# JustKshitijD/genomicsbench_palisade

Hardware: AMD Instinct MI355X
Metric: GCUPS (phmm) + Mreads/s (fmi) on 'large' set at 1/2/4/8 MI355X (higher is better)
Workload: dtype f32+f64 (phmm), int64 (fmi), int32/f64 (chain), int32 (bsw); 1 GPU; phmm large: 64 batches, 755118 testcases, 47.634 G cells per step (whole job); all 755118 testcases; 36.0% of rank 0's testcases on the f64 fallback; parallelism=shard1 (strong scaling, no data-path collective)

## Files before the change

### genomicsbench_palisade_amd/csrc/phmm.hip

```cpp
#include <hip/hip_runtime.h>

#include <algorithm>
#include <cmath>
#include <cstdint>
#include <cstdlib>
#include <chrono>
#include <cstring>
#include <functional>
#include <future>
#include <limits>
#include <mutex>
#include <string>
#include <unordered_map>
#include <thread>
#include <type_traits>
#include <vector>

#include "../../include/gb_phmm.h"
#include "gb_common.h"
#include "gb_common_wave.h"

namespace {

constexpr int kWave = 64;
constexpr int kLdsHaplen = 9400;
constexpr int kMaxHaplen = 65535;
constexpr int kBndPad = 72;
constexpr int kRecPad = 16;
constexpr int kQualTab = 128;
constexpr int kStackRows = 2048;
constexpr int kPlanBuckets = 128;
constexpr int kPlanCount = 8, kPlanCursor = kPlanCount + kPlanBuckets, kPlanTotal = kPlanCursor + kPlanBuckets;
constexpr int kCountWords = kPlanTotal + 8;
constexpr int kPredSampled = kPlanTotal + 1, kPredSamplePred = kPlanTotal + 2, kPredPredicted = kPlanTotal + 3;
constexpr int kPredConfirmed = kPlanTotal + 4, kPredRedone = kPlanTotal + 5, kRedoUnits = kPlanTotal + 6;
constexpr int kRedoNext = kPlanTotal + 7;
static_assert(kRedoNext < kCountWords, "counter words");
constexpr int kMaxF64Parts = 8;
constexpr int kM2M = ((127 * 128) >> 1) + 128;

constexpr int kMaxQual = 254;
constexpr double kJacTol = 8.0;
constexpr double kJacStep = 0.0001;
#define GB_JAC_INV_STEP (1.0 / kJacStep)
constexpr int kJacSize = (int)(kJacTol / kJacStep) + 1;

template <typename T>
struct HostTables {
  T ph2pr[kQualTab];
  T one_minus[kQualTab];
  T div3[kQualTab];
  T m2m[kM2M];
  T init_const;
  T log10_init;
};

template <typename T>
static int fast_round(T d) {
  return (d > (T)0.0) ? (int)(d + (T)0.5) : (int)(d - (T)0.5);
}

template <typename T>
static T log10sum(const std::vector<T> &jac, T small, T big) {
  if (small > big) std::swap(small, big);
  T diff = big - small;
  if (diff >= (T)kJacTol) return big;
  int ind = fast_round<T>((T)(diff * (T)GB_JAC_INV_STEP));
  return big + jac[ind];
}

template <typename T>
static void build_tables(HostTables<T> &t) {
  std::vector<T> jac(kJacSize);
  for (int k = 0; k < kJacSize; k++) jac[k] = (T)(log10(1.0 + pow(10.0, -((double)k) * kJacStep)));
  const double inv_ln10 = 1.0 / log(10);
  std::vector<T> m2m_full(((kMaxQual + 1) * (kMaxQual + 2)) >> 1);
  for (int i = 0, off = 0; i <= kMaxQual; off += ++i)
    for (int j = 0; j <= i; j++) {
      double s = log10sum<T>(jac, (T)(-0.1 * i), (T)(-0.1 * j));
      double l = log1p(-std::min(1.0, pow(10, s))) * inv_ln10;
      m2m_full[off + j] = (T)(pow(10, l));
    }
  for (int k = 0; k < kM2M; k++) t.m2m[k] = m2m_full[k];
  for (int x = 0; x < kQualTab; x++) {
    if constexpr (sizeof(T) == 4)
      t.ph2pr[x] = powf(10.f, -((float)x) / 10.f);
    else
      t.ph2pr[x] = pow(10.0, -((double)x) / 10.0);
    t.one_minus[x] = (T)1.0 - t.ph2pr[x];
    t.div3[x] = t.ph2pr[x] / (T)3.0;
  }
  if constexpr (sizeof(T) == 4) {
    t.init_const = ldexpf(1.f, 120);
    t.log10_init = log10f(t.init_const);
  } else {
    t.init_const = ldexp(1.0, 1020);
    t.log10_init = log10(t.init_const);
  }
}

static uint8_t base_code(char ch) {
  switch ((uint8_t)ch) {
    case 'A': return 0;
    case 'C': return 1;
    case 'T': return 2;
    case 'G': return 3;
    case 'N': return 4;
    default: return 0;
  }
}
static uint8_t read_match_mask(uint8_t rc) { return rc == 4 ? 0x1F : (uint8_t)((1u << rc) | 0x10); }

constexpr double kExitGrowthMax = 2.0;
constexpr uint8_t kMayExit = 0x80;
static double exit_growth(const HostTables<float> &t, const uint8_t *rec, int R) {
  const double inf = std::numeric_limits<double>::infinity();
  double G = 1.0;
  for (int k = 0; k + 1 < R; k++) {
    const int qd = rec[3 * R + k] & 127, qc = rec[4 * R + k] & 127;
    const int ni = rec[2 * R + k + 1] & 127, nd = rec[3 * R + k + 1] & 127, nc = rec[4 * R + k + 1] & 127;
    const int mn = std::min(ni, nd), mx = std::max(ni, nd);
    const double nMM = t.m2m[((mx * (mx + 1)) >> 1) + mn], nMX = t.ph2pr[ni];
    const double nGAPM = t.one_minus[nc], nXX = t.ph2pr[nc];
    const double pYY = t.ph2pr[qc], leak = (double)t.ph2pr[qd] * nGAPM;
    if (leak > 0 && pYY >= 1.0) return inf;
    const double gM = nMM + nMX + (leak > 0 ? leak / (1.0 - pYY) : 0.0), gX = nGAPM + nXX;
    const double g = std::max(gM, gX);
    if (g > 1.0) G *= g;
    if (G > 1e30) return inf;
  }
  return G;
}

constexpr double kCertMax = 2.0;
constexpr uint8_t kMayPredict = 0x80;
struct CertTab {
  double q[kQualTab];
  double p[kQualTab];
  double c[kQualTab];
  double m[kM2M];
};
static void build_cert_tab(const HostTables<float> &tf, const HostTables<double> &td, CertTab &T) {
  auto ratio = [](float f, double d) {
    return d > 0 ? std::max(1.0, (double)f / d) : (f > 0 ? std::numeric_limits<double>::infinity() : 1.0);
  };
  for (int x = 0; x < kQualTab; x++) {
    T.q[x] = std::max(ratio(tf.one_minus[x], td.one_minus[x]), ratio(tf.div3[x], td.div3[x]));
    T.p[x] = ratio(tf.ph2pr[x], td.ph2pr[x]);
    T.c[x] = std::max(T.p[x], ratio(tf.one_minus[x], td.one_minus[x]));
  }
  for (int k = 0; k < kM2M; k++) T.m[k] = ratio(tf.m2m[k], td.m2m[k]);
}
static double cert_log_rho(const CertTab &T, const uint8_t *q, const uint8_t *qi, const uint8_t *qd,
                           const uint8_t *qc, int R) {
  double rho = 1.0;
  for (int r = 0; r < R; r++) {
    const int a = q[r] & 127, i = qi[r] & 127, d = qd[r] & 127, c = qc[r] & 127;
    if (i <= 3 || d <= 3 || a == 0 || c == 0) return std::numeric_limits<double>::infinity();
    const int mn = std::min(i, d), mx = std::max(i, d), m = ((mx * (mx + 1)) >> 1) + mn;
    rho = std::max(rho, std::max(std::max(T.q[a], T.p[i]), std::max(std::max(T.p[d], T.c[c]), T.m[m])));
  }
  return std::log(rho);
}
__host__ __device__ inline double cert_K(double log_rho, int R, int C) {
  const double steps = (double)R + (double)C, D = 4.0 * steps + (double)C + 4.0;
  return exp((2.0 * steps + 2.0) * log_rho + D * 5.9604644e-8);
}

struct __attribute__((aligned(16))) TcDesc {
  uint32_t read_off;
  uint32_t hap_off;
  uint32_t dims;
  uint32_t out_idx;
};

template <typename T>
struct DevTab {
  const T *ph2pr, *one_minus, *div3, *m2m;
  T init_const;
};

template <typename T>
struct __attribute__((aligned(2 * sizeof(T)))) Brec {
  T z, w;
};

template <int (*F)(int, int)>
__device__ __forceinline__ float dpp(float v, float keep) {
  return __builtin_bit_cast(float, F(__builtin_bit_cast(int, v), __builtin_bit_cast(int, keep)));
}
template <int (*F)(int, int)>
__device__ __forceinline__ double dpp(double v, double keep) {
  long long vb = __builtin_bit_cast(long long, v), kb = __builtin_bit_cast(long long, keep);
  int lo = F((int)(vb & 0xffffffffll), (int)(kb & 0xffffffffll));
  int hi = F((int)(vb >> 32), (int)(kb >> 32));
  return __builtin_bit_cast(double, ((long long)hi << 32) | (unsigned int)lo);
}
template <int (*F)(int, int)>
__device__ __forceinline__ uint32_t dpp(uint32_t v, uint32_t keep) {
  return (uint32_t)F((int)v, (int)keep);
}

__device__ __forceinline__ float select_dist(uint32_t rmask, uint32_t h, float dmatch, float dmis) {
  uint32_t m = (uint32_t)__builtin_amdgcn_sbfe((int)rmask, h, 1);
  uint32_t r = (m & __builtin_bit_cast(uint32_t, dmatch)) | (~m & __builtin_bit_cast(uint32_t, dmis));
  return __builtin_bit_cast(float, r);
}
__device__ __forceinline__ double select_dist(uint32_t rmask, uint32_t h, double dmatch, double dmis) {
  uint32_t m;
  asm("v_bfe_i32 %0, %1, %2, 1" : "=v"(m) : "v"(rmask), "v"(h));
  const uint64_t a = __builtin_bit_cast(uint64_t, dmatch), b = __builtin_bit_cast(uint64_t, dmis);
  const uint32_t lo = (m & (uint32_t)a) | (~m & (uint32_t)b);
  const uint32_t hi = (m & (uint32_t)(a >> 32)) | (~m & (uint32_t)(b >> 32));
  return __builtin_bit_cast(double, ((uint64_t)hi << 32) | lo);
}

template <int O>
__device__ __forceinline__ float swz_xor(float v) {
  return __builtin_bit_cast(float, __builtin_amdgcn_ds_swizzle(__builtin_bit_cast(int, v), (O << 10) | 0x1F));
}
template <int O>
__device__ __forceinline__ double swz_xor(double v) {
  const long long b = __builtin_bit_cast(long long, v);
  const int lo = __builtin_amdgcn_ds_swizzle((int)(b & 0xffffffffll), (O << 10) | 0x1F);
  const int hi = __builtin_amdgcn_ds_swizzle((int)(b >> 32), (O << 10) | 0x1F);
  return __builtin_bit_cast(double, ((long long)hi << 32) | (unsigned int)lo);
}
template <typename T>
__device__ __forceinline__ T wave_sum_xor(T acc) {
  acc += __shfl_xor(acc, 32);
  acc += swz_xor<16>(acc);
  acc += swz_xor<8>(acc);
  acc += swz_xor<4>(acc);
  acc += swz_xor<2>(acc);
  acc += swz_xor<1>(acc);
  return acc;
}

__device__ __forceinline__ int fresh(int v) {
  asm volatile("" : "+v"(v));
  return v;
}

__device__ __forceinline__ uint32_t load_code(const uint8_t *p) {
  uint32_t h = *p;
  asm volatile("" : "+v"(h));
  return h;
}

template <typename T>
struct RowParams {
  T pMY, pYY, dmatch, dmis;
  T nMM, nGAPM, nGAPMx, nMX, nXX;
  uint32_t rmask;
};

template <typename T>
struct LaneState {
  T Mp, Yp, zo, wo, zd;
};

template <typename T, bool kSum, bool kWrite>
__device__ __forceinline__ void phmm_step(const Brec<T> &rec, uint32_t h, LaneState<T> &st,
// ... 609 lines not shown
      phmm_step2<T, kSum, W>(c1, h1, hb, A, B, PA, PB, sMa, sXa, sMb, sXb, wr + 1, last_lane);
      phmm_step2<T, kSum, W>(c2, h2, hb, A, B, PA, PB, sMa, sXa, sMb, sXb, wr + 2, last_lane);
      phmm_step2<T, kSum, W>(c3, h3, hb, A, B, PA, PB, sMa, sXa, sMb, sXb, wr + 3, last_lane);
    }
    for (; t < end; t++) single(t, wr_tag);
  };
  if constexpr (kWrite) {
    const int a = min(steps, kNoWrite2);
    run(0, a, std::false_type{});
    run(a, steps, std::true_type{});
  } else {
    run(0, steps, std::false_type{});
  }
}

template <typename T>
__device__ __forceinline__ void phmm_stack2(const Stack &S, const uint32_t *__restrict__ stk_tc,
                                            const TcDesc *__restrict__ descs, const uint8_t *__restrict__ pool,
                                            const DevTab<T> &tab, T *__restrict__ raw_out, uint8_t *smem_raw) {
  const int lane = threadIdx.x;
  const int C = (int)S.C;
  Brec<T> *bnd = reinterpret_cast<Brec<T> *>(smem_raw) + kRecPad;
  uint8_t *hcol = smem_raw + sizeof(Brec<T>) * (size_t)(C + kBndPad2 + kRecPad) + kCodePad2;
  const int na = (int)S.count;
  TcDesc d = {0, 0, 0, 0};
  if (lane < na) d = descs[stk_tc[S.first + lane]];
  const int rows = lane < na ? (int)(d.dims & 0xffff) + 2 : 0;
  const int incl = gb::scan_add(rows);
  const int T_rows = __builtin_amdgcn_readlane(incl, 63);
  const int e_start = incl - rows, e_R = rows - 2;
  const T init_Y = tab.init_const / (T)C;
  const uint8_t *hcode = pool + S.hap_off;
  for (int c = lane; c < C + kBndPad2; c += kWave) {
    Brec<T> b;
    b.z = (T)0;
    b.w = (T)0;
    bnd[c] = b;
  }
  for (int c = lane - kCodePad2; c < C + kBndPad2; c += kWave)
    hcol[c] = (c >= 1 && c <= C) ? hcode[c - 1] : (c == 0 ? 5 : (c < 0 ? 6 : 0));
  __syncthreads();

  const int nstripes = (T_rows + kRows2 - 1) / kRows2;
  for (int s = 0; s < nstripes; s++) {
    const int g0 = s * kRows2 + 2 * lane, g1 = g0 + 1;
    int lo = 0, hi = na - 1;
    while (__builtin_amdgcn_ballot_w64(lo < hi)) {
      const int mid = (lo + hi + 1) >> 1;
      const int sm = __shfl(e_start, mid);
      if (lo < hi) {
        if (sm <= g0) lo = mid; else hi = mid - 1;
      }
    }
    const int nxt = __shfl(e_start, min(lo + 1, kWave - 1));
    const int lob = (lo + 1 < na && nxt <= g1) ? lo + 1 : lo;
    const int sa = __shfl(e_start, lo), Ra = __shfl(e_R, lo);
    const uint32_t rda = (uint32_t)__shfl((int)d.read_off, lo), oa = (uint32_t)__shfl((int)d.out_idx, lo);
    const int sb = __shfl(e_start, lob), Rb = __shfl(e_R, lob);
    const uint32_t rdb = (uint32_t)__shfl((int)d.read_off, lob), ob = (uint32_t)__shfl((int)d.out_idx, lob);
    const int ra = g0 - sa, rb = g1 - sb;
    const bool deadA = g0 >= T_rows, deadB = g1 >= T_rows;
    RowParams<T> PA, PB;
    LaneState<T> A, B;
    const T z_top = lane == 0 ? bnd[0].z : (T)0;
    setup_row<T>(2 * lane, deadA, ra, Ra, pool + rda, tab, init_Y, z_top, PA, A);
    setup_row<T>(2 * lane + 1, deadB, rb, Rb, pool + rdb, tab, init_Y, (T)0, PB, B);
    const uint64_t pa = __builtin_amdgcn_ballot_w64(!deadA && ra == Ra + 1);
    const uint64_t pb = __builtin_amdgcn_ballot_w64(!deadB && rb == Rb + 1);
    const bool more = s < nstripes - 1;
    const int steps = more ? C + kRows2 - 1 : C + (T_rows - s * kRows2) - 1;
    T *outA = raw_out + oa, *outB = raw_out + ob;
    if (pa | pb) {
      if (more)
        phmm_stripe2<T, true, true>(steps, A, B, PA, PB, bnd, hcol, C, lane, pa, pb, outA, outB);
      else
        phmm_stripe2<T, true, false>(steps, A, B, PA, PB, bnd, hcol, C, lane, pa, pb, outA, outB);
    } else {
      phmm_stripe2<T, false, true>(steps, A, B, PA, PB, bnd, hcol, C, lane, 0, 0, outA, outB);
    }
    __syncthreads();
  }
}

template <int W>
__global__ __launch_bounds__(64) __attribute__((amdgpu_waves_per_eu(W ? W : 1, 8))) void phmm_forward2(
                                                     const Stack *__restrict__ stacks,
                                                     const uint32_t *__restrict__ stk_tc,
                                                     const TcDesc *__restrict__ descs,
                                                     const uint8_t *__restrict__ pool, DevTab<float> tab,
                                                     float *__restrict__ raw_out) {
  extern __shared__ __attribute__((aligned(16))) uint8_t smem_raw[];
  phmm_stack2<float>(stacks[blockIdx.x], stk_tc, descs, pool, tab, raw_out, smem_raw);
}

template <typename T, bool kF64Pass, bool kLong = false, bool kExit = false, bool kRedo = false>
__global__ __launch_bounds__(64) __attribute__((amdgpu_waves_per_eu(kLong ? 1 : (sizeof(T) == 4 ? 8 : 4), 8))) void phmm_forward(
    const Stack *__restrict__ stacks, int nstacks,
                                                    const uint32_t *__restrict__ stk_tc,
                                                    const TcDesc *__restrict__ descs,
                                                    const uint8_t *__restrict__ pool, DevTab<T> tab,
                                                    T *__restrict__ raw_out, const float *__restrict__ raw_f,
                                                    int *__restrict__ counter, int force, uint8_t *scratch,
                                                    size_t scratch_stride, const uint32_t *__restrict__ units,
                                                    const uint8_t *__restrict__ sel, int sel_want) {
  extern __shared__ __attribute__((aligned(16))) uint8_t smem_raw[];
  uint8_t *rec = kLong ? scratch + (size_t)blockIdx.x * scratch_stride : smem_raw;
  const bool roll = (force >> 16) & 1;
  if constexpr (kRedo) {
    const int nwork = __builtin_amdgcn_readfirstlane(counter[kRedoUnits]);
    while (true) {
      int k = 0;
      if (threadIdx.x == 0) k = atomicAdd(counter + kRedoNext, 1);
      k = __builtin_amdgcn_readfirstlane(__shfl(k, 0));
      if (k >= nwork) break;
      k = __builtin_amdgcn_readfirstlane((int)units[k]);
      phmm_stack<T, false, false, true>(stacks[k], stk_tc, descs, pool, tab, raw_out, nullptr, false, rec, 0, 1, nullptr,
                                        roll, sel, sel_want);
      __syncthreads();
    }
  } else if constexpr (kF64Pass || kLong) {
    int done = 0;
    int *next = counter + (kLong ? (kF64Pass ? 3 : 2) : 1);
    const int parts = (kF64Pass && !kLong) ? max(1, (force >> 8) & 0xFF) : 1;
    const int nwork = units ? __builtin_amdgcn_readfirstlane(counter[kPlanTotal]) : nstacks * parts;
    while (true) {
      int k = 0;
      if (threadIdx.x == 0) k = atomicAdd(next, 1);
      k = __builtin_amdgcn_readfirstlane(__shfl(k, 0));
      if (k >= nwork) break;
      if (units) k = __builtin_amdgcn_readfirstlane((int)units[k]);
      done += phmm_stack<T, kF64Pass, false, !kLong>(stacks[k / parts], stk_tc, descs, pool, tab, raw_out, raw_f,
                                                     (force & 0xFF) != 0, rec, k % parts, parts, nullptr, roll);
      __syncthreads();
    }
    if (kF64Pass && threadIdx.x == 0 && done) atomicAdd(counter, done);
  } else {
    phmm_stack<T, false, kExit, true>(stacks[blockIdx.x], stk_tc, descs, pool, tab, raw_out, nullptr, false, rec, 0, 1,
                                      reinterpret_cast<unsigned long long *>(counter + 4), roll, sel, sel_want);
  }
}

__global__ __launch_bounds__(256) void f64_plan(const Stack *__restrict__ stacks, int nunits, int parts,
                                                const uint32_t *__restrict__ stk_tc, const TcDesc *__restrict__ descs,
                                                const float *__restrict__ raw_f, int force, int roll,
                                                uint8_t *__restrict__ ukey, int *__restrict__ counter) {
  __shared__ int hist[kPlanBuckets];
  for (int i = threadIdx.x; i < kPlanBuckets; i += blockDim.x) hist[i] = 0;
  __syncthreads();
  const int u = blockIdx.x * blockDim.x + threadIdx.x;
  if (u < nunits) {
    const Stack S = stacks[u / parts];
    const int part = u % parts, lo = part * (int)S.count / parts, hi = (part + 1) * (int)S.count / parts;
    int rows = 0;
    for (int a = lo; a < hi; a++) {
      const TcDesc d = descs[stk_tc[S.first + a]];
      if (force || raw_f[d.out_idx] < 1e-28f) rows += (int)(d.dims & 0xffff) + 2;
    }
    int key = 0;
    if (rows) {
      key = (int)((stack_steps(rows, (int)S.C, kWave, roll != 0) + 63) / 64);
      key = key < 1 ? 1 : (key > kPlanBuckets - 1 ? kPlanBuckets - 1 : key);
      atomicAdd(&hist[key], 1);
    }
    ukey[u] = (uint8_t)key;
  }
  __syncthreads();
  for (int i = threadIdx.x; i < kPlanBuckets; i += blockDim.x)
    if (hist[i]) atomicAdd(&counter[kPlanCount + i], hist[i]);
}

__global__ __launch_bounds__(256) void f64_plan_order(int nunits, const uint8_t *__restrict__ ukey,
                                                      int *__restrict__ counter, uint32_t *__restrict__ units) {
  __shared__ int cnt[kPlanBuckets], off[kPlanBuckets], hist[kPlanBuckets], base[kPlanBuckets];
  for (int i = threadIdx.x; i < kPlanBuckets; i += blockDim.x) {
    cnt[i] = counter[kPlanCount + i];
    hist[i] = 0;
  }
  __syncthreads();
  if (threadIdx.x == 0) {
    int sum = 0;
    for (int k = kPlanBuckets - 1; k >= 1; k--) {
      off[k] = sum;
      sum += cnt[k];
    }
    if (blockIdx.x == 0) counter[kPlanTotal] = sum;
  }
  const int u = blockIdx.x * blockDim.x + threadIdx.x;
  const int key = u < nunits ? ukey[u] : 0;
  int rank = 0;
  if (key) rank = atomicAdd(&hist[key], 1);
  __syncthreads();
  for (int i = threadIdx.x; i < kPlanBuckets; i += blockDim.x)
    if (hist[i]) base[i] = atomicAdd(&counter[kPlanCursor + i], hist[i]);
  __syncthreads();
  if (key) units[off[key] + base[key] + rank] = (uint32_t)u;
}

constexpr int kPredMargin = -100, kPredThresh = 6412, kPredPad = 63;
constexpr int kPredMaxRows = 2046;
constexpr int kPlaneWords = 320;
constexpr int kPredChunks = 4;
constexpr int kGateDen = 8, kGateTake = 2, kGateAll = 1024;
constexpr int64_t kPredMinCells = 5000000000ll;
static_assert(kPlaneWords % 2 == 0 && kPlaneWords >= (kLdsHaplen + 64 + 256) / 32 + 3, "plane words");
enum PredictMode { kPredSample = 0, kPredAll = 2, kPredOpen = 3 };

__device__ __forceinline__ int pred_overhang(int n) { return n > 0 ? 350 + 100 * n : 0; }

__global__ __launch_bounds__(64) void phmm_predict(const Stack *__restrict__ stacks, int nstacks,
                                                   const uint32_t *__restrict__ stk_tc,
                                                   const TcDesc *__restrict__ descs, const uint8_t *__restrict__ pool,
                                                   float *__restrict__ raw_f, uint8_t *__restrict__ pred,
                                                   int *__restrict__ counter, int mode) {
  __shared__ uint32_t plane[4][kPlaneWords];
  const int lane = threadIdx.x;
  const int first = (int)blockIdx.x, stride = (int)gridDim.x;
  int seen = 0, npred = 0;
  for (int k = first; k < nstacks; k += stride) {
    const Stack S = stacks[k];
    const int C = (int)S.C;
    const int cnt = (int)S.count;
    if (mode == kPredSample && nstacks > kGateAll && ((S.first * 2654435761u) >> 28) != 0) continue;
    const int n_take = mode == kPredSample ? min(kGateTake, cnt) : cnt;
    const int a_first = mode == kPredSample ? (int)((S.first >> 4) % (uint32_t)cnt) : 0;
    const int a_step = mode == kPredSample ? (cnt + 1) / 2 : 1;
    seen += n_take;
    if (C > kLdsHaplen) continue;
    const uint8_t *hcode = pool + S.hap_off;
    const int nw = (C + 64 + 256) / 32 + 2;
    __syncthreads();
    for (int j = 0; 2 * j < nw; j++) {
      const int c = 64 * j + lane - 64;
      const uint32_t code = (c >= 0 && c < C) ? hcode[c] : 255u;
      uint64_t m[4];
      for (int b = 0; b < 4; b++) m[b] = __builtin_amdgcn_ballot_w64(code == (uint32_t)b || code >= 4u);
      if (lane < 8) {
        const uint64_t v = lane < 2 ? m[0] : lane < 4 ? m[1] : lane < 6 ? m[2] : m[3];
        plane[lane >> 1][2 * j + (lane & 1)] = (uint32_t)(v >> (32 * (lane & 1)));
      }
    }
    __syncthreads();
    const int lcC = [&]() {
      const int msb = 31 - __builtin_clz((uint32_t)C);
      const uint32_t l2 = ((uint32_t)msb << 8) | ((((uint32_t)C << (31 - msb)) >> 23) & 0xFFu);
      return (int)((l2 * 7706u) >> 16);
    }();
    const int thr = kPredThresh - lcC + kPredMargin;
    for (int j = 0; j < n_take; j++) {
      const int a = (a_first + j * a_step) % cnt;
      const TcDesc d = descs[stk_tc[S.first + a]];
      const int R = (int)(d.dims & 0xffff);
      const uint8_t *rb = pool + d.read_off;
      if (!(rb[R] & kMayPredict) || R > kPredMaxRows) continue;
      int best = 1 << 30;
      if (mode != kPredAll) {
        const int dhi = C - R + kPredPad;
        for (int g0 = 0; g0 - kPredPad <= dhi; g0 += 64 * kPredChunks) {
          const int nch = min(kPredChunks, (dhi + kPredPad - g0) / 64 + 1);
          const int e0 = 1 + g0 + lane;
          const uint32_t sh = (uint32_t)e0 & 31u;
          const uint32_t *w0 = &plane[0][e0 >> 5];
          uint32_t n0[kPredChunks], n1[kPredChunks], n2[kPredChunks];
          for (int c = 0; c < kPredChunks; c++) n0[c] = n1[c] = n2[c] = 0;
          for (int r64 = 0; r64 < R; r64 += 64) {
            const int row = r64 + lane;
            const bool in = row < R;
            const uint32_t rm = in ? rb[row] : 0u, qv = in ? (uint32_t)(rb[R + row] & 127) : 0u;
            uint64_t rp[4], qp[3];
            for (int b = 0; b < 4; b++) rp[b] = __builtin_amdgcn_ballot_w64((rm >> b) & 1u);
            qp[0] = __builtin_amdgcn_ballot_w64(in && qv < 14u);
            qp[1] = __builtin_amdgcn_ballot_w64(in && qv >= 14u && qv < 28u);
            qp[2] = __builtin_amdgcn_ballot_w64(in && qv >= 28u);
            const uint32_t *w = w0 + (r64 >> 5);
            const bool two = r64 + 32 < R;
#pragma unroll
            for (int c = 0; c < kPredChunks; c++) {
              if (c < nch) {
                uint32_t ha[4], hb[4];
#pragma unroll
                for (int p = 0; p < 4; p++) {
                  const uint32_t x0 = w[p * kPlaneWords + 2 * c], x1 = w[p * kPlaneWords + 2 * c + 1];
                  const uint32_t x2 = w[p * kPlaneWords + 2 * c + 2];
                  ha[p] = __builtin_amdgcn_alignbit(x1, x0, sh);
                  hb[p] = __builtin_amdgcn_alignbit(x2, x1, sh);
                }
                const uint32_t ma = ~(((uint32_t)rp[0] & ha[0]) | ((uint32_t)rp[1] & ha[1]) | ((uint32_t)rp[2] & ha[2]) |
                                      ((uint32_t)rp[3] & ha[3]));
                n0[c] += __builtin_popcount(ma & (uint32_t)qp[0]);
                n1[c] += __builtin_popcount(ma & (uint32_t)qp[1]);
                n2[c] += __builtin_popcount(ma & (uint32_t)qp[2]);
                if (two) {
                  const uint32_t mb = ~(((uint32_t)(rp[0] >> 32) & hb[0]) | ((uint32_t)(rp[1] >> 32) & hb[1]) |
                                        ((uint32_t)(rp[2] >> 32) & hb[2]) | ((uint32_t)(rp[3] >> 32) & hb[3]));
                  n0[c] += __builtin_popcount(mb & (uint32_t)(qp[0] >> 32));
                  n1[c] += __builtin_popcount(mb & (uint32_t)(qp[1] >> 32));
                  n2[c] += __builtin_popcount(mb & (uint32_t)(qp[2] >> 32));
                }
              }
            }
          }
#pragma unroll
          for (int c = 0; c < kPredChunks; c++) {
            const int dg = g0 + 64 * c + lane - kPredPad;
            if (c < nch && dg <= dhi) {
              const int n_lo = min(R, max(0, -dg)), n_hi = min(R - n_lo, max(0, R + dg - C));
              const int cost = 140 * (int)n0[c] + 250 * (int)n1[c] + 390 * (int)n2[c] + pred_overhang(n_lo) +
                               pred_overhang(n_hi);
              best = min(best, cost);
            }
          }
        }
        best = __builtin_amdgcn_readlane(gb::scan_min<(1 << 30)>(best), 63);
      }
      if (best > thr) {
        npred++;
        if (lane == 0 && mode != kPredSample) {
          pred[d.out_idx] = 1;
          raw_f[d.out_idx] = 0.f;
        }
      }
    }
  }
  if (lane == 0) {
    if (mode == kPredSample && seen) atomicAdd(counter + kPredSampled, seen);
    if (mode == kPredSample && npred) atomicAdd(counter + kPredSamplePred, npred);
    if (mode != kPredSample && npred) atomicAdd(counter + kPredPredicted, npred);
  }
}

__global__ __launch_bounds__(256) void phmm_verify(const TcDesc *__restrict__ descs, int n,
                                                   const uint8_t *__restrict__ pool,
                                                   const uint8_t *__restrict__ pred, const double *__restrict__ rd,
                                                   uint8_t *__restrict__ redo, int *__restrict__ counter) {
  if (__builtin_amdgcn_readfirstlane(counter[kPredPredicted]) == 0) return;
  int nok = 0, nre = 0;
  unsigned long long cells = 0;
  for (int k = blockIdx.x * blockDim.x + threadIdx.x; k < n; k += gridDim.x * blockDim.x) {
    if (!pred[k]) continue;
    const TcDesc d = descs[k];
    const int R = (int)(d.dims & 0xffff), C = (int)(d.dims >> 16);
    const uint8_t *lp = pool + d.read_off + 5 * (size_t)R;
    const uint32_t lb = (uint32_t)lp[0] | (uint32_t)lp[1] << 8 | (uint32_t)lp[2] << 16 | (uint32_t)lp[3] << 24;
    const double K = cert_K((double)__builtin_bit_cast(float, lb), R, C);
    if (rd[k] * 0x1p-900 * K + 4e-35 < (double)1e-28f) {
      cells += (unsigned long long)R * (unsigned long long)C;
      nok++;
    } else {
      redo[k] = 1;
      nre++;
    }
  }
  for (int o = 32; o >= 1; o >>= 1) {
    cells += __shfl_xor(cells, o);
    nok += __shfl_xor(nok, o);
    nre += __shfl_xor(nre, o);
  }
  if ((threadIdx.x & 63) == 0) {
    if (nok) {
      atomicAdd(counter + kPredConfirmed, nok);
      atomicAdd(reinterpret_cast<unsigned long long *>(counter + 4), (unsigned long long)nok);
      atomicAdd(reinterpret_cast<unsigned long long *>(counter + 4) + 1, cells);
    }
    if (nre) atomicAdd(counter + kPredRedone, nre);
  }
}

__global__ __launch_bounds__(256) void phmm_redo_plan(const Stack *__restrict__ stacks, int nstacks,
                                                      const uint32_t *__restrict__ stk_tc,
                                                      const uint8_t *__restrict__ redo, int *__restrict__ counter,
                                                      uint32_t *__restrict__ units) {
  if (__builtin_amdgcn_readfirstlane(counter[kPredRedone]) == 0) return;
  const int k = blockIdx.x * blockDim.x + threadIdx.x;
  if (k >= nstacks) return;
  const Stack S = stacks[k];
  bool any = false;
  for (uint32_t a = 0; a < S.count && !any; a++) any = redo[stk_tc[S.first + a]] != 0;
  if (any) units[atomicAdd(counter + kRedoUnits, 1)] = (uint32_t)k;
}

__global__ void phmm_warm(int *count) {
  if (threadIdx.x == 0 && blockIdx.x == 0) count[3] = 0;
}

__global__ void phmm_finalize(const float *__restrict__ rf, double *__restrict__ rd,
                              const uint8_t *__restrict__ redo, double *__restrict__ out, int n,
                              float log10_init_f, double log10_init_d, int *__restrict__ counter) {
  int i = blockIdx.x * blockDim.x + threadIdx.x;
  if (i >= n) return;
  if (redo && redo[i] && rf[i] >= 1e-28f) {
    rd[i] = 0.0;
    atomicSub(counter, 1);
  }
  out[i] = (rf[i] < 1e-28f) ? (log10(rd[i]) - log10_init_d) : (double)(log10f(rf[i]) - log10_init_f);
}

struct DeviceTables {
  int device = -1;
  float *f = nullptr;
  double *d = nullptr;
  HostTables<float> hf;
  HostTables<double> hd;
};

std::mutex g_mu;
HostTables<float> *g_hf = nullptr;
HostTables<double> *g_hd = nullptr;
CertTab *g_cert = nullptr;
std::unordered_map<int, DeviceTables *> g_dev;

int ensure_host_tables() {
  if (!g_hf) {
    auto *f = new HostTables<float>();
    auto *d = new HostTables<double>();
    build_tables(*f);
    build_tables(*d);
    auto *c = new CertTab();
    build_cert_tab(*f, *d, *c);
    g_cert = c;
    g_hf = f;
    g_hd = d;
  }
  return GB_OK;
}

template <typename T>
int upload_tables(const HostTables<T> &h, T **dst) {
  const size_t nel = 3 * kQualTab + kM2M;
  std::vector<T> blob(nel);
  std::memcpy(blob.data(), h.ph2pr, sizeof(T) * kQualTab);
  std::memcpy(blob.data() + kQualTab, h.one_minus, sizeof(T) * kQualTab);
  std::memcpy(blob.data() + 2 * kQualTab, h.div3, sizeof(T) * kQualTab);
  std::memcpy(blob.data() + 3 * kQualTab, h.m2m, sizeof(T) * kM2M);
  GB_HIP(hipMalloc(dst, sizeof(T) * nel));
  GB_HIP(hipMemcpy(*dst, blob.data(), sizeof(T) * nel, hipMemcpyHostToDevice));
  return GB_OK;
}

int get_device_tables(DeviceTables **out) {
  std::lock_guard<std::mutex> lk(g_mu);
  ensure_host_tables();
  int dev = -1;
  GB_HIP(hipGetDevice(&dev));
  auto it = g_dev.find(dev);
  if (it != g_dev.end()) {
    *out = it->second;
    return GB_OK;
  }
  auto *t = new DeviceTables();
  t->device = dev;
  t->hf = *g_hf;
  t->hd = *g_hd;
  int st = upload_tables(*g_hf, &t->f);
  if (st) return st;
  st = upload_tables(*g_hd, &t->d);
  if (st) return st;
  for (auto fn : {(const void *)phmm_forward<float, false>, (const void *)phmm_forward<float, false, false, true>,
                  (const void *)phmm_forward<double, true>,
                  (const void *)phmm_forward<float, false, false, false, true>, (const void *)phmm_forward2<0>, (const void *)phmm_forward2<6>, (const void *)phmm_forward2<8>})
    GB_HIP(hipFuncSetAttribute(fn, hipFuncAttributeMaxDynamicSharedMemorySize, 160 * 1024));
  g_dev[dev] = t;
  *out = t;
  return GB_OK;
}

template <typename T>
DevTab<T> dev_tab(const T *base, T init_const) {
  DevTab<T> t;
  t.ph2pr = base;
  t.one_minus = base + kQualTab;
  t.div3 = base + 2 * kQualTab;
  t.m2m = base + 3 * kQualTab;
  t.init_const = init_const;
  return t;
}

struct ReadKey {
  const char *rs, *q, *i, *d, *c;
  int len;
  bool operator==(const ReadKey &o) const {
    return rs == o.rs && q == o.q && i == o.i && d == o.d && c == o.c && len == o.len;
  }
};
struct HapKey {
  const char *h;
  int len;
  bool operator==(const HapKey &o) const { return h == o.h && len == o.len; }
};
struct KeyHash {
  size_t mix(size_t a, size_t b) const { return a ^ (b + 0x9e3779b97f4a7c15ull + (a << 6) + (a >> 2)); }
  size_t operator()(const ReadKey &k) const {
    size_t h = std::hash<const void *>()(k.rs);
    for (const void *p : {(const void *)k.q, (const void *)k.i, (const void *)k.d, (const void *)k.c})
      h = mix(h, std::hash<const void *>()(p));
    return mix(h, (size_t)k.len);
  }
  size_t operator()(const HapKey &k) const { return mix(std::hash<const void *>()(k.h), (size_t)k.len); }
};

}

struct gb_phmm_batch {
  DeviceTables *tabs = nullptr;
  hipStream_t stream = nullptr;
  hipEvent_t ev[4] = {nullptr, nullptr, nullptr, nullptr};
  int n = 0;
  int max_haplen = 0;
  int64_t cells = 0;
  gb::PinnedBuf<uint8_t> h_stage;
  gb::DevBuf<uint8_t> d_arena;
  TcDesc *d_desc = nullptr;
  gb::DevBuf<uint8_t> d_pool;
  float *d_rf = nullptr;
  double *d_rd = nullptr;
  double *d_out = nullptr;
  uint32_t *d_stk_tc = nullptr;
  Stack *d_stacks = nullptr;
  int nstacks = 0;
  int n_long = 0;
  int long_grid = 0;
  gb::DevBuf<uint8_t> d_scratch;
  size_t scratch_stride = 0;
  gb::DevBuf<int> d_count;
  uint32_t *d_units = nullptr;
  uint8_t *d_ukey = nullptr;
  int f64_grid = 0;
  int cus = 256;
  bool ran = false;
  bool force_f64 = false;
  int rpl = 1;
  int w2 = 0;
  int f64_parts = 2;
  bool f64_plan = true;
  bool f32_exit = true;
  bool roll = true;
  int predict = 1;
  bool resident = false;
  bool gate_open = false;
  int gate_n = 0, gate_pred = 0;
  uint8_t *d_pred = nullptr;
  uint8_t *d_redo = nullptr;
  size_t pred_bytes = 0;
  std::vector<uint32_t> hid;
  std::vector<Stack> stacks;
  std::vector<uint64_t> skeys;
  std::vector<std::vector<uint8_t>> pools;
};

namespace {
int warm_up(DeviceTables *t);
}

extern "C" {

int gb_phmm_init(void) {
  DeviceTables *t = nullptr;
  int st = get_device_tables(&t);
// ... 541 lines not shown
  clk.mark("chunk 0 filled");
  if ((st = gb_phmm_batch_run(B[0]))) return fail(st);
  launched = 1;
  int fetched = 0;
  for (int c = 1; c < k; c++) {
    const auto r = ready[c - 1].get();
    if (r.first) {
      gb::set_error("%s", r.second.c_str());
      return fail(r.first);
    }
    clk.mark("chunk ready");
    if ((st = gb_phmm_batch_run(B[c]))) return fail(st);
    launched = c + 1;
    if (c >= 2) {
      if ((st = fetch(fetched++))) return fail(st);
      clk.mark("chunk fetched");
    }
  }
  while (fetched < k)
    if ((st = fetch(fetched++))) return fail(st);
  clk.mark("last chunks fetched");
  return st;
}

}

extern "C" {

int gb_phmm_batch_create(const gb_testcase *tcs, int n, gb_phmm_batch **out) {
  GB_ARG(out, "gb_phmm_batch_create: null out");
  GB_ARG(n >= 0 && (n == 0 || tcs), "gb_phmm_batch_create: bad testcase array (n=%d)", n);
  *out = nullptr;
  DeviceTables *tabs = nullptr;
  int st = get_device_tables(&tabs);
  if (st) return st;
  gb_phmm_batch *b = nullptr;
  if ((st = batch_new(tabs, &b))) return st;
  b->resident = true;
  if ((st = batch_fill(b, tcs, n))) {
    gb_phmm_batch_destroy(b);
    return st;
  }
  *out = b;
  return GB_OK;
}

int gb_phmm_batch_run(gb_phmm_batch *b) {
  gb::Range range_("gb.phmm.batch_run");
  GB_ARG(b, "gb_phmm_batch_run: null batch");
  DeviceTables *t = b->tabs;
  GB_HIP(hipSetDevice(t->device));
  const int n = b->n;
  GB_HIP(hipEventRecord(b->ev[0], b->stream));
  GB_HIP(hipMemsetAsync(b->d_count, 0, kCountWords * sizeof(int), b->stream));
  const bool predict = n > 0 && b->gate_open && b->f32_exit && !b->force_f64 && b->rpl == 1 && b->nstacks > 0;
  GB_HIP(hipMemsetAsync(b->d_rd, 0, predict ? b->pred_bytes : sizeof(double) * std::max(n, 1), b->stream));
  if (n > 0) {
    const size_t rec = (size_t)(b->max_haplen + kBndPad + kRecPad), codes = (size_t)(b->max_haplen + kBndPad + kWave);
    const size_t lds_f = sizeof(Brec<float>) * rec + codes + 16;
    const size_t lds_d = sizeof(Brec<double>) * rec + codes + 16;
    auto f32k = phmm_forward<float, false>;
    auto f64k = phmm_forward<double, true>;
    const int ns = b->nstacks, nl = b->n_long;
    const Stack *d_long = b->d_stacks + ns;
    if (b->f32_exit) f32k = phmm_forward<float, false, false, true>;
    const uint8_t *skip = predict ? b->d_pred : nullptr;
    if (predict) {
      const int pg = std::min(ns, b->cus * 16);
      hipLaunchKernelGGL(phmm_predict, dim3(pg), dim3(kWave), 0, b->stream, b->d_stacks, ns, b->d_stk_tc, b->d_desc,
                         b->d_pool, b->d_rf, b->d_pred, b->d_count, b->predict == 2 ? (int)kPredAll : (int)kPredOpen);
      GB_HIP(hipGetLastError());
    }
    if (!b->force_f64) {
      if (ns > 0 && b->rpl == 2) {
        const size_t lds_f2 = sizeof(Brec<float>) * (size_t)(b->max_haplen + kBndPad2 + kRecPad) +
                              (size_t)(b->max_haplen + kBndPad2 + kCodePad2) + 16;
        auto k2 = b->w2 == 8 ? phmm_forward2<8> : b->w2 == 6 ? phmm_forward2<6> : phmm_forward2<0>;
        hipLaunchKernelGGL(k2, dim3(ns), dim3(kWave), lds_f2, b->stream, b->d_stacks, b->d_stk_tc,
                           b->d_desc, b->d_pool, dev_tab<float>(t->f, t->hf.init_const), b->d_rf);
      } else if (ns > 0) {
        hipLaunchKernelGGL(f32k, dim3(ns), dim3(kWave), lds_f, b->stream, b->d_stacks, ns, b->d_stk_tc, b->d_desc,
                           b->d_pool, dev_tab<float>(t->f, t->hf.init_const), b->d_rf, (const float *)nullptr,
                           b->d_count, b->roll ? 1 << 16 : 0, (uint8_t *)nullptr, (size_t)0, (const uint32_t *)nullptr,
                           skip, 0);
      }
      if (nl > 0)
        hipLaunchKernelGGL((phmm_forward<float, false, true>), dim3(b->long_grid), dim3(kWave), 0, b->stream, d_long,
                           nl, b->d_stk_tc, b->d_desc, b->d_pool, dev_tab<float>(t->f, t->hf.init_const), b->d_rf,
                           (const float *)nullptr, b->d_count, 0, b->d_scratch, b->scratch_stride,
                           (const uint32_t *)nullptr, (const uint8_t *)nullptr, 0);
      GB_HIP(hipGetLastError());
    }
    GB_HIP(hipEventRecord(b->ev[1], b->stream));
    if (ns > 0) {
      const int nunits = ns * b->f64_parts;
      const int g64 = std::min(nunits, b->f64_grid);
      if (b->f64_plan) {
        const dim3 pg((unsigned)((nunits + 255) / 256)), pb(256);
        hipLaunchKernelGGL(f64_plan, pg, pb, 0, b->stream, b->d_stacks, nunits, b->f64_parts, b->d_stk_tc, b->d_desc,
                           (const float *)b->d_rf, b->force_f64 ? 1 : 0, b->roll ? 1 : 0, b->d_ukey, b->d_count);
        hipLaunchKernelGGL(f64_plan_order, pg, pb, 0, b->stream, nunits, (const uint8_t *)b->d_ukey, b->d_count,
                           b->d_units);
      }
      hipLaunchKernelGGL(f64k, dim3(g64), dim3(kWave), lds_d, b->stream, b->d_stacks, ns, b->d_stk_tc, b->d_desc,
                         b->d_pool, dev_tab<double>(t->d, t->hd.init_const), b->d_rd, (const float *)b->d_rf,
                         b->d_count, (b->force_f64 ? 1 : 0) | (b->f64_parts << 8) | (b->roll ? 1 << 16 : 0),
                         (uint8_t *)nullptr, (size_t)0,
                         b->f64_plan ? (const uint32_t *)b->d_units : nullptr, (const uint8_t *)nullptr, 0);
    }
    if (nl > 0)
      hipLaunchKernelGGL((phmm_forward<double, true, true>), dim3(b->long_grid), dim3(kWave), 0, b->stream, d_long,
                         nl, b->d_stk_tc, b->d_desc, b->d_pool, dev_tab<double>(t->d, t->hd.init_const), b->d_rd,
                         (const float *)b->d_rf, b->d_count, b->force_f64 ? 1 : 0, b->d_scratch, b->scratch_stride,
                         (const uint32_t *)nullptr, (const uint8_t *)nullptr, 0);
    if (predict) {
      const dim3 sg((unsigned)((ns + 255) / 256)), tb(256);
      const dim3 vg((unsigned)std::min((n + 255) / 256, b->cus));
      hipLaunchKernelGGL(phmm_verify, vg, tb, 0, b->stream, (const TcDesc *)b->d_desc, n,
                         (const uint8_t *)b->d_pool.get(), (const uint8_t *)b->d_pred,
                         (const double *)b->d_rd, b->d_redo, b->d_count);
      hipLaunchKernelGGL(phmm_redo_plan, sg, tb, 0, b->stream, (const Stack *)b->d_stacks, ns,
                         (const uint32_t *)b->d_stk_tc, (const uint8_t *)b->d_redo, b->d_count, b->d_units);
      hipLaunchKernelGGL((phmm_forward<float, false, false, false, true>), dim3(std::min(ns, b->cus * 8)), dim3(kWave),
                         lds_f, b->stream, b->d_stacks, ns, b->d_stk_tc, b->d_desc, b->d_pool,
                         dev_tab<float>(t->f, t->hf.init_const), b->d_rf, (const float *)nullptr, b->d_count,
                         b->roll ? 1 << 16 : 0, (uint8_t *)nullptr, (size_t)0, (const uint32_t *)b->d_units,
                         (const uint8_t *)b->d_redo, 1);
    }
    GB_HIP(hipGetLastError());
    GB_HIP(hipEventRecord(b->ev[2], b->stream));
    hipLaunchKernelGGL(phmm_finalize, dim3((n + 255) / 256), dim3(256), 0, b->stream, b->d_rf, b->d_rd,
                       predict ? (const uint8_t *)b->d_redo : nullptr, b->d_out, n, t->hf.log10_init,
                       t->hd.log10_init, b->d_count);
    GB_HIP(hipGetLastError());
  } else {
    GB_HIP(hipEventRecord(b->ev[1], b->stream));
    GB_HIP(hipEventRecord(b->ev[2], b->stream));
  }
  GB_HIP(hipEventRecord(b->ev[3], b->stream));
  b->ran = true;
  return GB_OK;
}

int gb_phmm_batch_sync(gb_phmm_batch *b) {
  GB_ARG(b, "gb_phmm_batch_sync: null batch");
  GB_HIP(hipStreamSynchronize(b->stream));
  return GB_OK;
}

int gb_phmm_batch_results(gb_phmm_batch *b, double *results, float *raw_f, double *raw_d,
                          uint8_t *used_double, double *dev_results) {
  GB_ARG(b, "gb_phmm_batch_results: null batch");
  if (!b->ran) {
    gb::set_error("gb_phmm_batch_results: batch has not been run");
    return GB_ERR_STATE;
  }
  GB_HIP(hipSetDevice(b->tabs->device));
  GB_HIP(hipStreamSynchronize(b->stream));
  const int n = b->n;
  if (n == 0) return GB_OK;
  std::vector<float> rf_v;
  std::vector<double> rd_v;
  const float *rf;
  const double *rd;
  const size_t off_d = gb::round_up<size_t>(sizeof(float) * (size_t)n, 256);
  if (b->h_stage && b->h_stage.capacity() >= off_d + sizeof(double) * (size_t)n) {
    GB_HIP(hipMemcpyAsync(b->h_stage, b->d_rf, sizeof(float) * n, hipMemcpyDeviceToHost, b->stream));
    GB_HIP(hipMemcpyAsync(b->h_stage + off_d, b->d_rd, sizeof(double) * n, hipMemcpyDeviceToHost, b->stream));
    GB_HIP(hipStreamSynchronize(b->stream));
    rf = (const float *)b->h_stage.get();
    rd = (const double *)(b->h_stage + off_d);
  } else {
    rf_v.resize(n);
    rd_v.resize(n);
    GB_HIP(hipMemcpy(rf_v.data(), b->d_rf, sizeof(float) * n, hipMemcpyDeviceToHost));
    GB_HIP(hipMemcpy(rd_v.data(), b->d_rd, sizeof(double) * n, hipMemcpyDeviceToHost));
    rf = rf_v.data();
    rd = rd_v.data();
  }
  if (dev_results) GB_HIP(hipMemcpy(dev_results, b->d_out, sizeof(double) * n, hipMemcpyDeviceToHost));
  const float l10f = b->tabs->hf.log10_init;
  const double l10d = b->tabs->hd.log10_init;
  auto part = [&](int lo, int hi) {
    for (int k = lo; k < hi; k++) {
      const bool ud = rf[k] < 1e-28f;
      if (results) results[k] = ud ? (log10(rd[k]) - l10d) : (double)(log10f(rf[k]) - l10f);
      if (raw_f) raw_f[k] = rf[k];
      if (raw_d) raw_d[k] = rd[k];
      if (used_double) used_double[k] = ud ? 1 : 0;
    }
  };
  const int nt = n >= (1 << 16) ? (int)std::max(1u, std::min(8u, std::thread::hardware_concurrency())) : 1;
  return gb::parallel("gb_phmm_batch_results", nt,
                      [&](int t) { part((int)((int64_t)n * t / nt), (int)((int64_t)n * (t + 1) / nt)); });
}

int gb_phmm_batch_timing(gb_phmm_batch *b, float *f32_ms, float *f64_ms, float *total_ms) {
  GB_ARG(b && b->ran, "gb_phmm_batch_timing: batch has not been run");
  GB_HIP(hipEventSynchronize(b->ev[3]));
  float a = 0, c = 0, tot = 0;
  GB_HIP(hipEventElapsedTime(&a, b->ev[0], b->ev[1]));
  GB_HIP(hipEventElapsedTime(&c, b->ev[1], b->ev[2]));
  GB_HIP(hipEventElapsedTime(&tot, b->ev[0], b->ev[3]));
  if (f32_ms) *f32_ms = a;
  if (f64_ms) *f64_ms = c;
  if (total_ms) *total_ms = tot;
  return GB_OK;
}

int gb_phmm_batch_stats(gb_phmm_batch *b, int64_t *testcases, int64_t *cells, int64_t *n_f64) {
  GB_ARG(b, "gb_phmm_batch_stats: null batch");
// ... 149 lines not shown
```

Measured before the change: 1859 GCUPS (phmm).

## Fuse predicted-skip verification and f32 redo into the f64 pass kernel

Removes the separate verify, redo-plan and redo-forward kernels. Each f64 work unit now checks its predicted-skipped testcases itself and immediately reruns the f32 stripe for any that fail certification. This saves three launches and a global redo scan, at the cost of extra registers and code in the f64 kernel and some serialised f32 work inside it. The prediction kernel also stops scanning diagonal chunks early once no lane can stay under the cost threshold, replacing the full min-reduction with an any-below test.

```diff
diff --git a/genomicsbench_palisade_amd/csrc/phmm.hip b/genomicsbench_palisade_amd/csrc/phmm.hip
--- a/genomicsbench_palisade_amd/csrc/phmm.hip
+++ b/genomicsbench_palisade_amd/csrc/phmm.hip
@@ -33,9 +33,8 @@
 constexpr int kPlanCount = 8, kPlanCursor = kPlanCount + kPlanBuckets, kPlanTotal = kPlanCursor + kPlanBuckets;
 constexpr int kCountWords = kPlanTotal + 8;
 constexpr int kPredSampled = kPlanTotal + 1, kPredSamplePred = kPlanTotal + 2, kPredPredicted = kPlanTotal + 3;
-constexpr int kPredConfirmed = kPlanTotal + 4, kPredRedone = kPlanTotal + 5, kRedoUnits = kPlanTotal + 6;
-constexpr int kRedoNext = kPlanTotal + 7;
-static_assert(kRedoNext < kCountWords, "counter words");
+constexpr int kPredConfirmed = kPlanTotal + 4, kPredRedone = kPlanTotal + 5;
+static_assert(kPredRedone < kCountWords, "counter words");
 constexpr int kMaxF64Parts = 8;
 constexpr int kM2M = ((127 * 128) >> 1) + 128;
 
@@ -179,6 +178,17 @@
   const T *ph2pr, *one_minus, *div3, *m2m;
   T init_const;
 };
+
+template <typename T>
+__host__ __device__ inline DevTab<T> dev_tab(const T *base, T init_const) {
+  DevTab<T> t;
+  t.ph2pr = base;
+  t.one_minus = base + kQualTab;
+  t.div3 = base + 2 * kQualTab;
+  t.m2m = base + 3 * kQualTab;
+  t.init_const = init_const;
+  return t;
+}
 
 template <typename T>
 struct __attribute__((aligned(2 * sizeof(T)))) Brec {
@@ -954,6 +964,41 @@
   }
 }
 
+__device__ __attribute__((noinline)) double cert_K_call(double log_rho, int R, int C) { return cert_K(log_rho, R, C); }
+
+__device__ __forceinline__ bool verify_unit(const Stack &S, int part, int parts, const uint32_t *__restrict__ stk_tc,
+                                            const TcDesc *__restrict__ descs, const uint8_t *__restrict__ pool,
+                                            const uint8_t *__restrict__ pred, const double *rd, uint8_t *redo,
+                                            int &nok, int &nre, unsigned long long &okcells) {
+  const int lane = threadIdx.x;
+  bool act = lane < (int)S.count;
+  if (parts > 1) act = act && lane >= part * (int)S.count / parts && lane < (part + 1) * (int)S.count / parts;
+  bool ok = false, re = false;
+  unsigned long long cells = 0;
+  if (act) {
+    const TcDesc d = descs[stk_tc[S.first + lane]];
+    if (pred[d.out_idx]) {
+      const int R = (int)(d.dims & 0xffff), C = (int)(d.dims >> 16);
+      const uint8_t *lp = pool + d.read_off + 5 * (size_t)R;
+      const uint32_t lb = (uint32_t)lp[0] | (uint32_t)lp[1] << 8 | (uint32_t)lp[2] << 16 | (uint32_t)lp[3] << 24;
+      const double K = cert_K_call((double)__builtin_bit_cast(float, lb), R, C);
+      ok = rd[d.out_idx] * 0x1p-900 * K + 4e-35 < (double)1e-28f;
+      re = !ok;
+      if (ok) cells = (unsigned long long)R * (unsigned long long)C;
+      else redo[d.out_idx] = 1;
+    }
+  }
+  const uint64_t okm = __builtin_amdgcn_ballot_w64(ok), rem = __builtin_amdgcn_ballot_w64(re);
+  if (okm) {
+    for (int o = 32; o >= 1; o >>= 1) cells += __shfl_xor(cells, o);
+    okcells += (unsigned long long)__builtin_amdgcn_readfirstlane((int)(cells & 0xffffffffu)) |
+               (unsigned long long)__builtin_amdgcn_readfirstlane((int)(cells >> 32)) << 32;
+    nok += __builtin_popcountll(okm);
+  }
+  nre += __builtin_popcountll(rem);
+  return rem != 0;
+}
+
 template <int W>
 __global__ __launch_bounds__(64) __attribute__((amdgpu_waves_per_eu(W ? W : 1, 8))) void phmm_forward2(
                                                      const Stack *__restrict__ stacks,
@@ -965,33 +1010,24 @@
   phmm_stack2<float>(stacks[blockIdx.x], stk_tc, descs, pool, tab, raw_out, smem_raw);
 }
 
-template <typename T, bool kF64Pass, bool kLong = false, bool kExit = false, bool kRedo = false>
+template <typename T, bool kF64Pass, bool kLong = false, bool kExit = false>
 __global__ __launch_bounds__(64) __attribute__((amdgpu_waves_per_eu(kLong ? 1 : (sizeof(T) == 4 ? 8 : 4), 8))) void phmm_forward(
     const Stack *__restrict__ stacks, int nstacks,
                                                     const uint32_t *__restrict__ stk_tc,
                                                     const TcDesc *__restrict__ descs,
                                                     const uint8_t *__restrict__ pool, DevTab<T> tab,
-                                                    T *__restrict__ raw_out, const float *__restrict__ raw_f,
+                                                    T *__restrict__ raw_out, const float *raw_f,
                                                     int *__restrict__ counter, int force, uint8_t *scratch,
                                                     size_t scratch_stride, const uint32_t *__restrict__ units,
-                                                    const uint8_t *__restrict__ sel, int sel_want) {
+                                                    const uint8_t *__restrict__ sel, int sel_want,
+                                                    const float *tabf, uint8_t *redo) {
   extern __shared__ __attribute__((aligned(16))) uint8_t smem_raw[];
   uint8_t *rec = kLong ? scratch + (size_t)blockIdx.x * scratch_stride : smem_raw;
   const bool roll = (force >> 16) & 1;
-  if constexpr (kRedo) {
-    const int nwork = __builtin_amdgcn_readfirstlane(counter[kRedoUnits]);
-    while (true) {
-      int k = 0;
-      if (threadIdx.x == 0) k = atomicAdd(counter + kRedoNext, 1);
-      k = __builtin_amdgcn_readfirstlane(__shfl(k, 0));
-      if (k >= nwork) break;
-      k = __builtin_amdgcn_readfirstlane((int)units[k]);
-      phmm_stack<T, false, false, true>(stacks[k], stk_tc, descs, pool, tab, raw_out, nullptr, false, rec, 0, 1, nullptr,
-                                        roll, sel, sel_want);
-      __syncthreads();
-    }
-  } else if constexpr (kF64Pass || kLong) {
+  if constexpr (kF64Pass || kLong) {
     int done = 0;
+    int nok = 0, nre = 0;
+    unsigned long long okcells = 0;
     int *next = counter + (kLong ? (kF64Pass ? 3 : 2) : 1);
     const int parts = (kF64Pass && !kLong) ? max(1, (force >> 8) & 0xFF) : 1;
     const int nwork = units ? __builtin_amdgcn_readfirstlane(counter[kPlanTotal]) : nstacks * parts;
@@ -1001,11 +1037,32 @@
       k = __builtin_amdgcn_readfirstlane(__shfl(k, 0));
       if (k >= nwork) break;
       if (units) k = __builtin_amdgcn_readfirstlane((int)units[k]);
-      done += phmm_stack<T, kF64Pass, false, !kLong>(stacks[k / parts], stk_tc, descs, pool, tab, raw_out, raw_f,
-                                                     (force & 0xFF) != 0, rec, k % parts, parts, nullptr, roll);
+      const int nf = phmm_stack<T, kF64Pass, false, !kLong>(stacks[k / parts], stk_tc, descs, pool, tab, raw_out, raw_f,
+                                                            (force & 0xFF) != 0, rec, k % parts, parts, nullptr, roll);
+      done += nf;
       __syncthreads();
-    }
-    if (kF64Pass && threadIdx.x == 0 && done) atomicAdd(counter, done);
+      if constexpr (kF64Pass && !kLong) {
+        if (sel && nf) {
+          if (verify_unit(stacks[k / parts], k % parts, parts, stk_tc, descs, pool, sel, raw_out, redo, nok, nre,
+                          okcells)) {
+            __syncthreads();
+            phmm_stack<float, false, false, true>(stacks[k / parts], stk_tc, descs, pool, dev_tab(tabf, 0x1p120f),
+                                                  const_cast<float *>(raw_f), nullptr, false, rec, k % parts, parts,
+                                                  nullptr, roll, redo, 1);
+            __syncthreads();
+          }
+        }
+      }
+    }
+    if (kF64Pass && threadIdx.x == 0) {
+      if (done) atomicAdd(counter, done);
+      if (nok) {
+        atomicAdd(counter + kPredConfirmed, nok);
+        atomicAdd(reinterpret_cast<unsigned long long *>(counter + 4), (unsigned long long)nok);
+        atomicAdd(reinterpret_cast<unsigned long long *>(counter + 4) + 1, okcells);
+      }
+      if (nre) atomicAdd(counter + kPredRedone, nre);
+    }
   } else {
     phmm_stack<T, false, kExit, true>(stacks[blockIdx.x], stk_tc, descs, pool, tab, raw_out, nullptr, false, rec, 0, 1,
                                       reinterpret_cast<unsigned long long *>(counter + 4), roll, sel, sel_want);
@@ -1124,17 +1181,25 @@
       const int R = (int)(d.dims & 0xffff);
       const uint8_t *rb = pool + d.read_off;
       if (!(rb[R] & kMayPredict) || R > kPredMaxRows) continue;
-      int best = 1 << 30;
+      bool low = false;
       if (mode != kPredAll) {
         const int dhi = C - R + kPredPad;
-        for (int g0 = 0; g0 - kPredPad <= dhi; g0 += 64 * kPredChunks) {
+        for (int g0 = 0; g0 - kPredPad <= dhi && !low; g0 += 64 * kPredChunks) {
           const int nch = min(kPredChunks, (dhi + kPredPad - g0) / 64 + 1);
           const int e0 = 1 + g0 + lane;
           const uint32_t sh = (uint32_t)e0 & 31u;
           const uint32_t *w0 = &plane[0][e0 >> 5];
           uint32_t n0[kPredChunks], n1[kPredChunks], n2[kPredChunks];
           for (int c = 0; c < kPredChunks; c++) n0[c] = n1[c] = n2[c] = 0;
-          for (int r64 = 0; r64 < R; r64 += 64) {
+          auto at_or_below = [&](int c) {
+            const int dg = g0 + 64 * c + lane - kPredPad;
+            const int n_lo = min(R, max(0, -dg)), n_hi = min(R - n_lo, max(0, R + dg - C));
+            const int cost = 140 * (int)n0[c] + 250 * (int)n1[c] + 390 * (int)n2[c] + pred_overhang(n_lo) +
+                             pred_overhang(n_hi);
+            return dg <= dhi && cost <= thr;
+          };
+          uint32_t alive = (1u << nch) - 1u;
+          for (int r64 = 0; r64 < R && alive; r64 += 64) {
             const int row = r64 + lane;
             const bool in = row < R;
             const uint32_t rm = in ? rb[row] : 0u, qv = in ? (uint32_t)(rb[R + row] & 127) : 0u;
@@ -1147,7 +1212,7 @@
             const bool two = r64 + 32 < R;
 #pragma unroll
             for (int c = 0; c < kPredChunks; c++) {
-              if (c < nch) {
+              if ((alive >> c) & 1u) {
                 uint32_t ha[4], hb[4];
 #pragma unroll
                 for (int p = 0; p < 4; p++) {
@@ -1170,21 +1235,19 @@
                 }
               }
             }
+            if (r64 + 64 < R) {
+#pragma unroll
+              for (int c = 0; c < kPredChunks; c++)
+                if (((alive >> c) & 1u) && !__builtin_amdgcn_ballot_w64(at_or_below(c))) alive &= ~(1u << c);
+            }
           }
 #pragma unroll
-          for (int c = 0; c < kPredChunks; c++) {
-            const int dg = g0 + 64 * c + lane - kPredPad;
-            if (c < nch && dg <= dhi) {
-              const int n_lo = min(R, max(0, -dg)), n_hi = min(R - n_lo, max(0, R + dg - C));
-              const int cost = 140 * (int)n0[c] + 250 * (int)n1[c] + 390 * (int)n2[c] + pred_overhang(n_lo) +
-                               pred_overhang(n_hi);
-              best = min(best, cost);
-            }
-          }
+          for (int c = 0; c < kPredChunks; c++)
+            if ((alive >> c) & 1u) low = low || at_or_below(c);
+          low = __builtin_amdgcn_ballot_w64(low) != 0;
         }
-        best = __builtin_amdgcn_readlane(gb::scan_min<(1 << 30)>(best), 63);
-      }
-      if (best > thr) {
+      }
+      if (!low) {
         npred++;
         if (lane == 0 && mode != kPredSample) {
           pred[d.out_idx] = 1;
@@ -1198,56 +1261,6 @@
     if (mode == kPredSample && npred) atomicAdd(counter + kPredSamplePred, npred);
     if (mode != kPredSample && npred) atomicAdd(counter + kPredPredicted, npred);
   }
-}
-
-__global__ __launch_bounds__(256) void phmm_verify(const TcDesc *__restrict__ descs, int n,
-                                                   const uint8_t *__restrict__ pool,
-                                                   const uint8_t *__restrict__ pred, const double *__restrict__ rd,
-                                                   uint8_t *__restrict__ redo, int *__restrict__ counter) {
-  if (__builtin_amdgcn_readfirstlane(counter[kPredPredicted]) == 0) return;
-  int nok = 0, nre = 0;
-  unsigned long long cells = 0;
-  for (int k = blockIdx.x * blockDim.x + threadIdx.x; k < n; k += gridDim.x * blockDim.x) {
-    if (!pred[k]) continue;
-    const TcDesc d = descs[k];
-    const int R = (int)(d.dims & 0xffff), C = (int)(d.dims >> 16);
-    const uint8_t *lp = pool + d.read_off + 5 * (size_t)R;
-    const uint32_t lb = (uint32_t)lp[0] | (uint32_t)lp[1] << 8 | (uint32_t)lp[2] << 16 | (uint32_t)lp[3] << 24;
-    const double K = cert_K((double)__builtin_bit_cast(float, lb), R, C);
-    if (rd[k] * 0x1p-900 * K + 4e-35 < (double)1e-28f) {
-      cells += (unsigned long long)R * (unsigned long long)C;
-      nok++;
-    } else {
-      redo[k] = 1;
-      nre++;
-    }
-  }
-  for (int o = 32; o >= 1; o >>= 1) {
-    cells += __shfl_xor(cells, o);
-    nok += __shfl_xor(nok, o);
-    nre += __shfl_xor(nre, o);
-  }
-  if ((threadIdx.x & 63) == 0) {
-    if (nok) {
-      atomicAdd(counter + kPredConfirmed, nok);
-      atomicAdd(reinterpret_cast<unsigned long long *>(counter + 4), (unsigned long long)nok);
-      atomicAdd(reinterpret_cast<unsigned long long *>(counter + 4) + 1, cells);
-    }
-    if (nre) atomicAdd(counter + kPredRedone, nre);
-  }
-}
-
-__global__ __launch_bounds__(256) void phmm_redo_plan(const Stack *__restrict__ stacks, int nstacks,
-                                                      const uint32_t *__restrict__ stk_tc,
-                                                      const uint8_t *__restrict__ redo, int *__restrict__ counter,
-                                                      uint32_t *__restrict__ units) {
-  if (__builtin_amdgcn_readfirstlane(counter[kPredRedone]) == 0) return;
-  const int k = blockIdx.x * blockDim.x + threadIdx.x;
-  if (k >= nstacks) return;
-  const Stack S = stacks[k];
-  bool any = false;
-  for (uint32_t a = 0; a < S.count && !any; a++) any = redo[stk_tc[S.first + a]] != 0;
-  if (any) units[atomicAdd(counter + kRedoUnits, 1)] = (uint32_t)k;
 }
 
 __global__ void phmm_warm(int *count) {
@@ -1327,23 +1340,11 @@
   st = upload_tables(*g_hd, &t->d);
   if (st) return st;
   for (auto fn : {(const void *)phmm_forward<float, false>, (const void *)phmm_forward<float, false, false, true>,
-                  (const void *)phmm_forward<double, true>,
-                  (const void *)phmm_forward<float, false, false, false, true>, (const void *)phmm_forward2<0>, (const void *)phmm_forward2<6>, (const void *)phmm_forward2<8>})
+                  (const void *)phmm_forward<double, true>, (const void *)phmm_forward2<0>, (const void *)phmm_forward2<6>, (const void *)phmm_forward2<8>})
     GB_HIP(hipFuncSetAttribute(fn, hipFuncAttributeMaxDynamicSharedMemorySize, 160 * 1024));
   g_dev[dev] = t;
   *out = t;
   return GB_OK;
-}
-
-template <typename T>
-DevTab<T> dev_tab(const T *base, T init_const) {
-  DevTab<T> t;
-  t.ph2pr = base;
-  t.one_minus = base + kQualTab;
-  t.div3 = base + 2 * kQualTab;
-  t.m2m = base + 3 * kQualTab;
-  t.init_const = init_const;
-  return t;
 }
 
 struct ReadKey {
@@ -2051,13 +2052,13 @@
         hipLaunchKernelGGL(f32k, dim3(ns), dim3(kWave), lds_f, b->stream, b->d_stacks, ns, b->d_stk_tc, b->d_desc,
                            b->d_pool, dev_tab<float>(t->f, t->hf.init_const), b->d_rf, (const float *)nullptr,
                            b->d_count, b->roll ? 1 << 16 : 0, (uint8_t *)nullptr, (size_t)0, (const uint32_t *)nullptr,
-                           skip, 0);
+                           skip, 0, (const float *)nullptr, (uint8_t *)nullptr);
       }
       if (nl > 0)
         hipLaunchKernelGGL((phmm_forward<float, false, true>), dim3(b->long_grid), dim3(kWave), 0, b->stream, d_long,
                            nl, b->d_stk_tc, b->d_desc, b->d_pool, dev_tab<float>(t->f, t->hf.init_const), b->d_rf,
                            (const float *)nullptr, b->d_count, 0, b->d_scratch, b->scratch_stride,
-                           (const uint32_t *)nullptr, (const uint8_t *)nullptr, 0);
+                           (const uint32_t *)nullptr, (const uint8_t *)nullptr, 0, (const float *)nullptr, (uint8_t *)nullptr);
       GB_HIP(hipGetLastError());
     }
     GB_HIP(hipEventRecord(b->ev[1], b->stream));
@@ -2075,27 +2076,14 @@
                          b->d_pool, dev_tab<double>(t->d, t->hd.init_const), b->d_rd, (const float *)b->d_rf,
                          b->d_count, (b->force_f64 ? 1 : 0) | (b->f64_parts << 8) | (b->roll ? 1 << 16 : 0),
                          (uint8_t *)nullptr, (size_t)0,
-                         b->f64_plan ? (const uint32_t *)b->d_units : nullptr, (const uint8_t *)nullptr, 0);
+                         b->f64_plan ? (const uint32_t *)b->d_units : nullptr, skip, 0,
+                         (const float *)t->f, predict ? b->d_redo : nullptr);
     }
     if (nl > 0)
       hipLaunchKernelGGL((phmm_forward<double, true, true>), dim3(b->long_grid), dim3(kWave), 0, b->stream, d_long,
                          nl, b->d_stk_tc, b->d_desc, b->d_pool, dev_tab<double>(t->d, t->hd.init_const), b->d_rd,
                          (const float *)b->d_rf, b->d_count, b->force_f64 ? 1 : 0, b->d_scratch, b->scratch_stride,
-                         (const uint32_t *)nullptr, (const uint8_t *)nullptr, 0);
-    if (predict) {
-      const dim3 sg((unsigned)((ns + 255) / 256)), tb(256);
-      const dim3 vg((unsigned)std::min((n + 255) / 256, b->cus));
-      hipLaunchKernelGGL(phmm_verify, vg, tb, 0, b->stream, (const TcDesc *)b->d_desc, n,
-                         (const uint8_t *)b->d_pool.get(), (const uint8_t *)b->d_pred,
-                         (const double *)b->d_rd, b->d_redo, b->d_count);
-      hipLaunchKernelGGL(phmm_redo_plan, sg, tb, 0, b->stream, (const Stack *)b->d_stacks, ns,
-                         (const uint32_t *)b->d_stk_tc, (const uint8_t *)b->d_redo, b->d_count, b->d_units);
-      hipLaunchKernelGGL((phmm_forward<float, false, false, false, true>), dim3(std::min(ns, b->cus * 8)), dim3(kWave),
-                         lds_f, b->stream, b->d_stacks, ns, b->d_stk_tc, b->d_desc, b->d_pool,
-                         dev_tab<float>(t->f, t->hf.init_const), b->d_rf, (const float *)nullptr, b->d_count,
-                         b->roll ? 1 << 16 : 0, (uint8_t *)nullptr, (size_t)0, (const uint32_t *)b->d_units,
-                         (const uint8_t *)b->d_redo, 1);
-    }
+                         (const uint32_t *)nullptr, (const uint8_t *)nullptr, 0, (const float *)nullptr, (uint8_t *)nullptr);
     GB_HIP(hipGetLastError());
     GB_HIP(hipEventRecord(b->ev[2], b->stream));
     hipLaunchKernelGGL(phmm_finalize, dim3((n + 255) / 256), dim3(256), 0, b->stream, b->d_rf, b->d_rd,
```

After: 1919 GCUPS (phmm), median of 6. 1.03x the previous value.
